# open-mmlab/Amphion

Measured on AMD Instinct MI355X. Metric: audio samples/sec (HiFi-GAN V1 22.05 kHz generator, mel->wav), higher is better.
Workload: dtype f32 (split-f16 MFMA: 3 x v_mfma_f32_32x32x16_f16 per term, f32 accumulate)

## Files before the change

amphion_amd/_lib.py:

```python
from __future__ import annotations

import ctypes
import os
import weakref
from ctypes import POINTER, c_char_p, c_float, c_int, c_int32, c_int64, c_size_t, c_void_p

_HERE = os.path.dirname(os.path.abspath(__file__))
LIB_PATH = os.environ.get("AMP_LIB_PATH") or os.path.join(_HERE, "lib", "libamphion_hip.so")

AMP_MAX_STAGES = 8
AMP_MAX_KERNELS = 8
AMP_MAX_DILATIONS = 8

AMP_ARCH_HIFIGAN, AMP_ARCH_BIGVGAN, AMP_ARCH_HIFIGAN_VITS = 0, 1, 2
AMP_ACT_LRELU, AMP_ACT_SNAKE, AMP_ACT_SNAKEBETA = 0, 1, 2
AMP_PRECISION_F32, AMP_PRECISION_F16X3 = 0, 1
AMP_CONV_OPT_PAD_REFLECT, AMP_CONV_OPT_TANH = 1, 2
AMP_PAD_REPLICATE, AMP_PAD_ZEROS, AMP_PAD_REFLECT = 0, 1, 2
AMP_PW_BIAS, AMP_PW_BIAS_GELU, AMP_PW_SCALE_RES = 0, 1, 2
PRECISIONS = {"f32": AMP_PRECISION_F32, "fp32": AMP_PRECISION_F32, "f16x3": AMP_PRECISION_F16X3}


class AmpError(RuntimeError):

# ... 109 lines not shown
    "amp_add_channel_bias": (c_int, [c_void_p, c_void_p, c_int, c_int, c_int, c_void_p]),
    "amp_layer_norm_c_ragged": (c_int, [c_void_p, c_void_p, c_void_p, c_void_p, c_void_p, c_void_p, c_int, c_int, c_int, c_float, c_int, c_void_p, c_void_p]),
    "amp_dds_seam": (c_int, [c_void_p, c_void_p, c_void_p, c_void_p, c_float, c_void_p, c_void_p, c_int, c_int, c_void_p, c_void_p, c_float,
                             c_void_p, c_int, c_int, c_int, c_void_p, c_void_p, c_void_p]),
    "amp_dwconv_layer_norm_c": (c_int, [c_void_p, c_void_p, c_void_p, c_int, c_int, c_void_p, c_void_p, c_void_p, c_int, c_int, c_int, c_float, c_int, c_void_p, c_void_p]),
    "amp_rel_attention_strided": (c_int, [c_void_p, c_void_p, c_void_p, ctypes.c_longlong, c_void_p, c_void_p, c_void_p, c_int, c_int, c_int, c_int, c_int, c_void_p, c_void_p]),
    "amp_set_rel_attention_tiled": (c_int, [c_int]),
    "amp_set_resblock_streams": (c_int, [c_int]),
    "amp_gen_prepare_streams": (c_int, [c_void_p]),
    "amp_rel_attention": (c_int, [c_void_p, c_void_p, c_void_p, c_void_p, c_void_p, c_void_p, c_int, c_int, c_int, c_int, c_int, c_void_p, c_void_p]),
    "amp_dwconv": (c_int, [c_void_p, c_void_p, c_void_p, c_void_p, c_int, c_int, c_int, c_int, c_int, c_void_p, c_void_p]),
    "amp_spline_flow": (c_int, [c_void_p, c_void_p, c_void_p, c_int, c_int, c_int, c_int, c_float, c_int, c_int, c_int, c_void_p, c_void_p]),
    "amp_spline_flow_proj": (c_int, [c_void_p, c_void_p, c_void_p, c_void_p, c_void_p, c_int, c_int, c_int, c_int, c_int, c_float, c_int, c_int, c_int, c_void_p, c_void_p]),
    "amp_affine_reverse": (c_int, [c_void_p, c_void_p, c_void_p, c_void_p, c_int, c_int, c_int, c_void_p, c_void_p]),
    "amp_embed_tokens": (c_int, [c_void_p, c_void_p, c_void_p, c_int, c_int, c_int, c_int, c_float, c_void_p, c_void_p]),
    "amp_durations": (c_int, [c_void_p, c_void_p, c_int, c_int, c_float, c_void_p, c_void_p, c_void_p, c_void_p]),
    "amp_expand_path": (c_int, [c_void_p, c_void_p, c_void_p, c_void_p, c_int, c_int, c_int, c_int, c_void_p, c_void_p, c_void_p]),
    "amp_expand_path_strided": (c_int, [c_void_p, ctypes.c_longlong, c_void_p, c_void_p, c_void_p, c_int, c_int, c_int, c_int, c_void_p, c_void_p, c_void_p]),
    "amp_gauss_sample": (c_int, [c_void_p, c_void_p, c_void_p, c_size_t, c_float, c_void_p, c_void_p]),
    "amp_snake": (c_int, [c_void_p, c_int, c_int, c_int, c_void_p, c_void_p, c_int, c_void_p, c_void_p]),
    "amp_fir_upsample": (c_int, [c_void_p, c_int, c_int, c_int, c_void_p, c_int, c_int, c_void_p, c_void_p]),
    "amp_fir_filter": (c_int, [c_void_p, c_int, c_int, c_int, c_void_p, c_int, c_int, c_int, c_int, c_int, c_void_p, c_void_p]),
    "amp_wav_to_pcm16": (c_int, [c_void_p, c_int, c_int, ctypes.c_longlong, c_void_p, c_void_p, ctypes.c_longlong, c_void_p]),
    "amp_conv_set_option": (c_int, [c_void_p, c_int, c_int]),
    "amp_pair_forward": (c_int, [c_void_p, c_void_p, c_void_p, c_int, c_int, c_float, c_void_p, c_void_p]),
    "amp_resblock_forward": (c_int, [POINTER(c_void_p), POINTER(c_void_p), c_int, c_void_p, c_int, c_int, c_float, c_void_p, c_void_p]),
    "amp_set_resblock_fusion": (c_int, [c_int]),
    "amp_conv_destroy": (None, [c_void_p]),
    "amp_set_small_conv": (c_int, [c_int]),
    "amp_set_conv_blk": (c_int, [c_int]),
    "amp_set_conv_rg_fast": (c_int, [c_int]),
    "amp_set_pingpong": (c_int, [c_int]),
    "amp_set_conv_blk_narrow": (c_int, [c_int]),
    "amp_ampblock_forward": (c_int, [POINTER(c_void_p), POINTER(c_void_p), c_int, c_void_p, c_void_p, c_int, c_void_p, c_void_p,
                                     c_void_p, c_int, c_int, c_void_p, c_int, c_float, c_void_p]),
    "amp_set_ampblock_fusion": (c_int, [c_int]),
    "amp_conv_create_gated": (c_int, [c_int, c_int, c_int, c_int, c_void_p, c_void_p, POINTER(c_void_p)]),
    "amp_wn_forward": (c_int, [POINTER(c_void_p), POINTER(c_void_p), c_int, c_void_p, c_void_p, ctypes.c_longlong, c_void_p, c_int, c_int,
                               c_void_p, c_void_p, c_void_p]),
    "amp_wn_gate": (c_int, [c_void_p, c_void_p, ctypes.c_longlong, c_void_p, c_int, c_int, c_int, c_void_p]),
    "amp_wn_accumulate": (c_int, [c_void_p, c_void_p, c_void_p, c_void_p, c_int, c_int, c_int, c_int, c_int, c_void_p]),
    "amp_sequence_mask": (c_int, [c_void_p, c_void_p, c_int, c_int, c_int, c_void_p]),
    "amp_coupling_apply": (c_int, [c_void_p, c_void_p, c_void_p, c_int, c_int, c_int, c_int, c_void_p]),
    "amp_flip_channels": (c_int, [c_void_p, c_void_p, c_int, c_int, c_int, c_void_p]),
    "amp_posterior_sample": (c_int, [c_void_p, c_void_p, c_void_p, c_void_p, c_int, c_int, c_int, c_void_p]),
    "amp_antialias_snake": (c_int, [c_void_p, c_int, c_int, c_int, c_void_p, c_void_p, c_int, c_void_p, c_void_p, c_void_p, c_void_p]),
    "amp_istft_forward": (c_int, [POINTER(amp_mel_desc), c_void_p, c_void_p, c_int, c_int, c_void_p, c_void_p, c_void_p, c_void_p, c_void_p]),
    "amp_mel_num_frames": (c_int, [POINTER(amp_mel_desc), c_int]),
    "amp_mel_init": (c_int, []),
    "amp_mel_forward_ragged": (c_int, [POINTER(amp_mel_desc), c_void_p, c_void_p, c_int, c_int, c_void_p, c_void_p, c_void_p, c_void_p, c_void_p, c_void_p, c_void_p]),
    "amp_mel_backward": (c_int, [POINTER(amp_mel_desc), c_void_p, c_int, c_int] + [c_void_p] * 11),
    "amp_mel_forward": (c_int, [POINTER(amp_mel_desc), c_void_p, c_int, c_int, c_void_p, c_void_p, c_void_p, c_void_p, c_void_p, c_void_p, c_void_p]),
}

EXPORTED_SYMBOLS = tuple(_SIGNATURES)

_lib = None


def lib():
    global _lib
    if _lib is None:
        if not os.path.exists(LIB_PATH):
            raise RuntimeError(
                f"{LIB_PATH} not found: build it with `python -m amphion_amd.build` "
                "(the HIP path has no CPU fallback)"
# ... 99 lines not shown
```

amphion_amd/build.py:

```python
from __future__ import annotations

import os
import subprocess
import sys
from concurrent.futures import ThreadPoolExecutor

HERE = os.path.dirname(os.path.abspath(__file__))
CSRC = os.path.join(HERE, "csrc")
OBJ = os.path.join(CSRC, "_build")
LIB = os.path.join(HERE, "lib", "libamphion_hip.so")
INCLUDE = os.path.join(os.path.dirname(HERE), "include")
HIPCC = os.environ.get("HIPCC", "/opt/rocm/bin/hipcc")
TAG = os.environ.get("AMP_BUILD_TAG", "")
if TAG:
    OBJ = os.path.join(CSRC, "_build_" + TAG)
    LIB = os.path.join(HERE, "lib", "libamphion_hip_" + TAG + ".so")
ARCH = "gfx950"
CONV_TAPS = (1, 2, 3, 5, 7, 11)
PAIR_TAPS = (3, 5, 7, 11)
SMALL_TAPS = (1, 3, 5, 7, 11)
BLK_TAPS = (2, 3, 7, 11)
RB_TAPS = (3, 5, 7, 11)
AMPB_TAPS = (3, 5, 7, 11)

FLAGS = ["--offload-arch=" + ARCH, "-O3", "-std=c++17", "-fPIC", "-I" + INCLUDE, "-I" + CSRC, "-Wall",
         "-Wno-unused-function"] + os.environ.get("AMP_BUILD_FLAGS", "").split()


def _units():
    units = [("runtime.hip", "runtime.o", []), ("conv_host.hip", "conv_host.o", []), ("generator.hip", "generator.o", []),
             ("ops_abi.hip", "ops_abi.o", []), ("small_kernels.hip", "small_kernels.o", []),
             ("mel.hip", "mel.o", []), ("vits_text.hip", "vits_text.o", []), ("pair3_f16x3.hip", "pair3_f16x3.o", []),
             ("conv_small3_f16x3.hip", "conv_small3_f16x3.o", []),
             ("pw_f16x3.hip", "pw_f16x3.o", []), ("dw_layer_f16x3.hip", "dw_layer_f16x3.o", []), ("diffwave.hip", "diffwave.o", [])]
    for kt in CONV_TAPS:
        units.append(("conv_mfma.hip", f"conv_mfma_kt{kt}.o", [f"-DAMP_KT={kt}"]))
        units.append(("conv_f16x3.hip", f"conv_f16x3_kt{kt}.o", [f"-DAMP_KT={kt}"]))
    for kt in BLK_TAPS:
        units.append(("conv_blk_f16x3.hip", f"conv_blk_f16x3_kt{kt}.o", [f"-DAMP_KT={kt}"]))
    for kt in SMALL_TAPS:
        units.append(("conv_small_f16x3.hip", f"conv_small_f16x3_kt{kt}.o", [f"-DAMP_KT={kt}"]))
    for kt in PAIR_TAPS:
        units.append(("pair_f16x3.hip", f"pair_f16x3_kt{kt}.o", [f"-DAMP_KT={kt}"]))
        units.append(("pair_strip_f16x3.hip", f"pair_strip_f16x3_kt{kt}.o", [f"-DAMP_KT={kt}"]))
    for kt in RB_TAPS:
        units.append(("rb_f16x3.hip", f"rb_f16x3_kt{kt}.o", [f"-DAMP_KT={kt}"]))
    for kt in AMPB_TAPS:
        units.append(("ampb_f16x3.hip", f"ampb_f16x3_kt{kt}.o", [f"-DAMP_KT={kt}"]))
    return units


def _deps_mtime():
    m = 0.0
    for root in (CSRC, INCLUDE):
        for fn in os.listdir(root):
            if fn.endswith((".h", ".hip", ".cpp")):
                m = max(m, os.path.getmtime(os.path.join(root, fn)))
    return max(m, os.path.getmtime(__file__))


def _compile(unit):
    src, obj, extra = unit
    cmd = [HIPCC] + FLAGS + extra + ["-c", os.path.join(CSRC, src), "-o", os.path.join(OBJ, obj)]
    r = subprocess.run(cmd, capture_output=True, text=True)
    if r.returncode != 0:
        raise RuntimeError("hipcc failed: " + " ".join(cmd) + "\n" + r.stdout + r.stderr)
    return obj


def build(force: bool = False, verbose: bool = False) -> str:
    os.makedirs(OBJ, exist_ok=True)
    os.makedirs(os.path.dirname(LIB), exist_ok=True)
# ... 18 lines not shown
```

amphion_amd/csrc/amp_host.h:

```cpp
#pragma once
#include <math.h>

#include <vector>

#include "amp_internal.h"

#define AMP_HIP(expr)                                                                  \
    do {                                                                               \
        hipError_t e__ = (expr);                                                       \
        if (e__ != hipSuccess) {                                                       \
            set_error("%s failed: %s (%s:%d)", #expr, hipGetErrorString(e__), __FILE__, __LINE__); \
            return AMP_ERR_HIP;                                                        \
        }                                                                              \
    } while (0)

#define AMP_RC(expr) do { int rc__ = (expr); if (rc__ != AMP_OK) return rc__; } while (0)

struct amp_conv {
    int transposed = 0, cin = 0, cout = 0, k = 0, stride = 1, dilation = 1, padding = 0;
    int M = 0, ntaps = 0, KT = 0, off0 = 0, dstep = 0, halo_left = 0, halo_right = 0, up = 1, up_pad = 0;
    int nchunks = 0;
    int precision = amp::PREC_F32;
    int pad_reflect = 0, tanh_out = 0;
    int gated_H = 0;
    int Mpad = 0;
    float wscale = 1.f;
    amp::ConvPlan plan{};
    void* wp_dev = nullptr;
    float* bias_dev = nullptr;
    ~amp_conv() {
        if (wp_dev) (void)hipFree(wp_dev);
        if (bias_dev) (void)hipFree(bias_dev);
    }
};

namespace amp {

int device_upload(const void* host, size_t bytes, void** out);

int default_precision();

constexpr int kConvBlkDefault = 3;
constexpr int kConvRgFastDefault = 1;
constexpr int kPingPongDefault = 1;
struct Config {
    int pair_strips = -1;
    int rb_fusion = 1;
    int ampb_fusion = 1;
    int conv_blk = kConvBlkDefault;
    size_t group_bytes = 0;
    int small_conv = 1;
    int conv_rg_fast = 1;
    int pingpong = 1;
    int narrow_blk = 1;
    int rb_streams = -1;
    Config();
};
Config& cfg();

struct RangeGuard {
    unsigned* dev = nullptr;
    unsigned* host = nullptr;
    hipEvent_t ev = nullptr;
    bool pending = false;
};
bool guard_init(RangeGuard& g);
void guard_free(RangeGuard& g);
int range_poll(RangeGuard* g, hipStream_t st);
int range_publish(RangeGuard* g, hipStream_t st);
int range_check_sync(RangeGuard* g, hipStream_t st, const char* who);
struct RangeFlagScope {
    explicit RangeFlagScope(unsigned* word);
    ~RangeFlagScope();
    RangeFlagScope(const RangeFlagScope&) = delete;
    RangeFlagScope& operator=(const RangeFlagScope&) = delete;
};

inline float pow2_weight_scale(float wmax) {
    int e2 = 0;
    if (wmax > 0.f) { (void)frexpf(wmax, &e2); if (ldexpf(1.f, e2 - 1) == wmax) e2 -= 1; }
    return wmax > 0.f ? ldexpf(1.f, 13 - e2) : 1.f;
}

template <class View>
std::vector<_Float16> pack_a_f16x3(int row_blocks, int k16, int taps, size_t pad_entries, float wscale, View view) {
    std::vector<_Float16> wp(((size_t)row_blocks * k16 * taps * 2 + pad_entries) * 64 * 8, (_Float16)0.f);
    for (int mb = 0; mb < row_blocks; ++mb)
// ... 46 lines not shown
```

amphion_amd/csrc/amp_internal.h:

```cpp
#pragma once
#include <hip/hip_runtime.h>
#include <stdarg.h>
#include <stdint.h>
#include <stdio.h>

#include <atomic>
#include <mutex>
#include <string>
#include <vector>

#include "amphion_hip.h"

namespace amp {

constexpr int KC = 8;
constexpr int KC16 = 16;

enum { PREC_F32 = 0, PREC_F16X3 = 1 };

struct ConvArgs {
    const float* x;
    const void* wp;
    const float* bias;
    const float* res;
    float* y;
    int B, Cin, Tin;
    long long xbs;
    int nchunks;
    int M;
    int Tq;
    int tiles_per_item;
    int rev;
    int row_groups;
    int off0, dstep;
    int halo_left;
    int wd;
    int Cout, Tout;
    int up, up_pad;
    float slope_in, slope_out;
    int mode;
    float div;
    float acc_scale, inv_scale;
    const int* lens;
    int len_mul;
    unsigned* range_flag;
    int pad_reflect;
    int tanh_out;
    int Mpad;
    const float* gate_cond;
    long long gate_cond_bs;
    int wn_H;
    float* wn_x;
    float* wn_out;
    int wn_first, wn_last;
};

struct PairArgs {
    const float* x;
    float* y;
    const void* wp1;
    const float* bias1;
    const void* wp2;
    const float* bias2;
    int B, C, T;
    int tiles_per_item;
    int strip_len;
    int strips_per_item;
    int wide;
    int rev;
    int dil;
    float slope;
    float sc1, isc1, sc2, isc2;
    int mode;
    float div;
    const int* lens;
    int len_mul;
    unsigned* range_flag;
};

struct ConvSmall3Args {
    ConvArgs a[3];
    int nx[3], ny[3];
};
hipError_t launch_conv_small3(const ConvSmall3Args& p, const int ni[3], hipStream_t stream);

struct Pair3Args {
    PairArgs a[3];
// ... 57 lines not shown
    const float* skip_in;
    float* x_out;
    float* skip_out;
    const uint4* wp1;
    const uint4* wp2;
    const float* w1f;
    const float* w2f;
    const float* bias1;
    const float* bias2;
    int C, n_mel, L, d;
    int K16;
    int tiles_per_item;
    float inv1, inv2;
    unsigned* range_flag;
};
size_t dw_layer_lds_bytes(int C, int n_mel, bool f32);
hipError_t launch_dw_layer(DwLayerArgs a, int B, bool f32, hipStream_t stream);

struct ConvPlan {
    int KT;
    int WM, WN;
    int NI;
    int HALO;
    int NT() const { return 32 * NI * WN; }
    int Mgroup() const { return 32 * WM; }
};

bool choose_plan(int ntaps, int M, int halo_total, int Tq, ConvPlan* plan);

template <int KT> hipError_t launch_conv(const ConvPlan& plan, const ConvArgs& a, hipStream_t stream);
template <int KT> hipError_t launch_conv_f16x3(const ConvPlan& plan, const ConvArgs& a, hipStream_t stream);
template <int KT> int conv_blk_nt(int cm, int halo_total);
template <int KT> hipError_t launch_conv_blk(int cm, int wn, const ConvArgs& a, hipStream_t stream);
constexpr int kSmallConvMaxChunks = 16;
template <int KT> hipError_t launch_conv_small(int ni, int epi, const ConvArgs& a, hipStream_t stream);
template <int KT> int pair_tile(int C, int dil);
template <int KT> hipError_t launch_pair(const PairArgs& a, hipStream_t stream);
template <int KT> int strip_step(int C, int dil, int wide, int* wg_per_cu);
template <int KT> hipError_t launch_strip(const PairArgs& a, hipStream_t stream);
template <int KT> int rb_tile(int C, int max_dil, int wide);
template <int KT> hipError_t launch_rb(const RbArgs& a, int wide, hipStream_t stream);
template <int KT> int ampb_tile(int C, int max_dil, int wide);
template <int KT> hipError_t launch_ampb(const AmpbArgs& a, int wide, hipStream_t stream);

hipError_t launch_conv_post(const float* x, const float* w_dev , const float* bias_dev ,
                            float* y, int B, int Cin, int T, int K, float slope_in, int apply_tanh,
                            const int* lens, int len_mul, hipStream_t stream);

hipError_t launch_act1d(const float* x, float* y, int B, int C, int T, const float* a_dev, const float* invb_dev,
                        const float* filt_up12, const float* filt_dn12, const int* lens, int len_mul,
                        hipStream_t stream, int rev = 0 );

hipError_t launch_add_channel_bias(float* y, const float* cb, int B, int C, int T, hipStream_t stream);
constexpr int AMP_MRF_MAX_PARTS = 3;
struct MrfSumArgs {
    float* y;
    const float* p[AMP_MRF_MAX_PARTS];
    int n;
    float div;
    size_t count;
};
hipError_t launch_mrf_sum(const MrfSumArgs& a, hipStream_t stream);

hipError_t launch_wn_gate(const float* a, const float* cond, long long cond_bs, float* out, int B, int H, int T,
                          hipStream_t stream);
hipError_t launch_wn_accumulate(float* x, float* out, const float* rs, const int* lens, int B, int H, int T, int last,
// ... 84 lines not shown
```

amphion_amd/csrc/conv_host.hip:

```cpp
#include <string.h>

#include <memory>
#include <type_traits>
#include <vector>

#include "amp_host.h"

namespace amp {

template <int... K> struct Taps { static constexpr int list[] = {K...}; };
using ConvTaps = Taps<1, 2, 3, 5, 7, 11>;
using BlkTaps = Taps<2, 3, 7, 11>;
using SmallTaps = Taps<1, 3, 5, 7, 11>;
using PairTaps = Taps<3, 5, 7, 11>;
using RbTaps = Taps<3, 5, 7, 11>;
using AmpbTaps = Taps<3, 5, 7, 11>;

template <int... K, typename R, typename F>
static R with_taps(Taps<K...>, int k, R dflt, F&& f) {
    R r = dflt;
    (void)((k == K && (r = f(std::integral_constant<int, K>{}), true)) || ...);
    return r;
}

static hipError_t launch_conv(const ConvPlan& p, const ConvArgs& a, hipStream_t s) {
    return with_taps(ConvTaps{}, p.KT, hipErrorInvalidValue, [&](auto K) { return launch_conv<K>(p, a, s); });
}
static hipError_t launch_conv_f16x3(const ConvPlan& p, const ConvArgs& a, hipStream_t s) {
    return with_taps(ConvTaps{}, p.KT, hipErrorInvalidValue, [&](auto K) { return launch_conv_f16x3<K>(p, a, s); });
}
static int conv_blk_nt(int k, int cm, int halo) { return with_taps(BlkTaps{}, k, 0, [&](auto K) { return conv_blk_nt<K>(cm, halo); }); }
static hipError_t launch_conv_blk(int k, int cm, int wn, const ConvArgs& a, hipStream_t s) {
    return with_taps(BlkTaps{}, k, hipErrorInvalidValue, [&](auto K) { return launch_conv_blk<K>(cm, wn, a, s); });
}
static hipError_t launch_conv_small(int k, int ni, int epi, const ConvArgs& a, hipStream_t s) {
    return with_taps(SmallTaps{}, k, hipErrorInvalidValue, [&](auto K) { return launch_conv_small<K>(ni, epi, a, s); });
}
static int pair_tile(int k, int C, int dil) { return with_taps(PairTaps{}, k, 0, [&](auto K) { return pair_tile<K>(C, dil); }); }
static hipError_t launch_pair(int k, const PairArgs& a, hipStream_t s) {
    return with_taps(PairTaps{}, k, hipErrorInvalidValue, [&](auto K) { return launch_pair<K>(a, s); });
}
static int strip_step(int k, int C, int dil, int wide, int* wg) {
    return with_taps(PairTaps{}, k, 0, [&](auto K) { return strip_step<K>(C, dil, wide, wg); });
}
static hipError_t launch_strip(int k, const PairArgs& a, hipStream_t s) {
    return with_taps(PairTaps{}, k, hipErrorInvalidValue, [&](auto K) { return launch_strip<K>(a, s); });
}
static int rb_tile(int k, int C, int max_dil, int wide) { return with_taps(RbTaps{}, k, 0, [&](auto K) { return rb_tile<K>(C, max_dil, wide); }); }
static hipError_t launch_rb(int k, const RbArgs& a, int wide, hipStream_t s) {
    return with_taps(RbTaps{}, k, hipErrorInvalidValue, [&](auto K) { return launch_rb<K>(a, wide, s); });
}
static int ampb_tile(int k, int C, int max_dil, int wide) {
    return with_taps(AmpbTaps{}, k, 0, [&](auto K) { return ampb_tile<K>(C, max_dil, wide); });
}
static hipError_t launch_ampb(int k, const AmpbArgs& a, int wide, hipStream_t s) {
    return with_taps(AmpbTaps{}, k, hipErrorInvalidValue, [&](auto K) { return launch_ampb<K>(a, wide, s); });
}

static int round_up_taps(int ntaps) {
    for (int kt : ConvTaps::list)
        if (kt >= ntaps) return kt;
    return -1;
}

bool choose_plan(int KT, int M, int halo_total, int , ConvPlan* plan) {
    bool ok = false;
// ... 24 lines not shown
        if ((long)(spi - 1) * L >= T) continue;
        const long steps = (L + hb + n1 - 1) / n1;
        const long rounds = ((long)B * spi + slots - 1) / slots;
        const long cost = rounds * (4 * steps + 1);
        if (best < 0 || cost < best) { best = cost; best_spi = spi; }
    }
    *spi_out = best_spi;
    *strip_len = (T + best_spi - 1) / best_spi;
}

static void strip_geometry(int B, int T, int n1, int hb, int wg_per_cu, int steps, bool ragged, int* strip_len, int* spi) {
    strip_plan(B, T, n1, hb, wg_per_cu, strip_len, spi);
    if (steps > 0 && steps * n1 - hb < T) { *strip_len = steps * n1 - hb; *spi = (T + *strip_len - 1) / *strip_len; }
    if (steps == 1 && !ragged && 4 * n1 - hb < T) {
        const int len4 = 4 * n1 - hb, spi4 = (T + len4 - 1) / len4;
        if ((long long)B * spi4 >= 1024) { *strip_len = len4; *spi = spi4; }
    }
}

constexpr long long kSmallGridWorkgroups = 384;

static bool small_conv_enabled() { return cfg().small_conv != 0; }

static int conv_blk_mode() { return cfg().conv_blk; }
static int narrow_blk_mode() { return cfg().narrow_blk; }
constexpr size_t kConvRgFastMaxWeightBytes = 3u << 20;
static bool conv_rg_fast() { return cfg().conv_rg_fast != 0; }
static thread_local unsigned g_launch_parity = 0;
int next_rev(const int* lens) {
    if (!cfg().pingpong || lens) return 0;
    return (int)(g_launch_parity++ & 1u);
}
constexpr long long kConvBlkMinWorkgroups = 512;

int conv_build(amp_conv* c, const float* w, const float* bias) {
    if (c->cin <= 0 || c->cout <= 0 || c->k <= 0 || c->stride <= 0 || c->dilation <= 0) {
        set_error("amp_conv: bad dimensions cin=%d cout=%d k=%d stride=%d dilation=%d", c->cin, c->cout, c->k, c->stride,
                  c->dilation);
        return AMP_ERR_INVALID;
    }
    if (!c->transposed) {
        if (c->stride != 1) { set_error("amp_conv: strided Conv1d is not on the vocoder path"); return AMP_ERR_UNSUPPORTED; }
        c->up = 1; c->up_pad = 0;
        c->M = c->cout;
        c->ntaps = c->k;
        c->off0 = -c->padding;
        c->dstep = c->dilation;
    } else if (c->stride == 1) {
        if (c->dilation != 1) { set_error("amp_conv: dilated ConvTranspose1d unsupported (dilation=%d)", c->dilation); return AMP_ERR_UNSUPPORTED; }
        c->up = 1; c->up_pad = 0;
        c->M = c->cout;
        c->ntaps = c->k;
        c->off0 = -(c->k - 1 - c->padding);
        c->dstep = 1;
    } else {
        if (c->dilation != 1) { set_error("amp_conv: dilated ConvTranspose1d unsupported (dilation=%d)", c->dilation); return AMP_ERR_UNSUPPORTED; }
        c->up = c->stride; c->up_pad = c->padding;
        c->M = c->cout * c->stride;
        c->ntaps = (c->k + c->stride - 1) / c->stride;
        c->off0 = 0;
        c->dstep = -1;
    }
    c->KT = round_up_taps(c->ntaps);
    if (c->KT < 0) { set_error("amp_conv: k=%d at stride=%d is %d taps, unsupported (max 11)", c->k, c->stride, c->ntaps); return AMP_ERR_UNSUPPORTED; }
    const int omin = c->dstep >= 0 ? c->off0 : c->off0 + (c->KT - 1) * c->dstep;
    const int omax = c->dstep >= 0 ? c->off0 + (c->KT - 1) * c->dstep : c->off0;
// ... 85 lines not shown
    a.pad_reflect = c->pad_reflect; a.tanh_out = c->tanh_out;
    a.range_flag = c->precision == PREC_F16X3 ? range_flag_for_current_device() : nullptr;
    a.rev = c->precision == PREC_F16X3 ? next_rev(lens) : 0;
    if (c->pad_reflect && (c->halo_left >= T || c->halo_right >= T)) {
        set_error("amp_conv_forward: reflection padding %d needs more than %d input samples", c->halo_left > c->halo_right ? c->halo_left : c->halo_right, T);
        return AMP_ERR_INVALID;
    }
    if (c->gated_H) { set_error("amp_conv_forward: a gated conv (amp_conv_create_gated) only runs inside amp_wn_forward"); return AMP_ERR_STATE; }
    if (c->precision == PREC_F16X3 && slope_in > 1.f) {
        set_error("amp_conv_forward: leaky_relu slope %g > 1 on the input is outside the f16x3 kernels (use AMP_PRECISION_F32)", (double)slope_in);
        return AMP_ERR_UNSUPPORTED;
    }
    tl_conv_transposed = c->transposed;
    if (c->precision == PREC_F32) {
        if (plan_small) return AMP_ERR_UNSUPPORTED;
        a.acc_scale = a.inv_scale = 1.f;
        AMP_HIP(launch_conv(plan, a, stream));
    } else {
        a.acc_scale = 16.f * c->wscale;
        a.inv_scale = 1.f / a.acc_scale;
        const long long wgs_half = (long long)B * ((a.Tq + 63) / 64) * ((c->M + plan.Mgroup() - 1) / plan.Mgroup());
        int blk_cm = 0, blk_nt = 0, blk_wn = 1;
        const bool blk_kt = c->KT == 2 || c->KT == 3 || (conv_blk_mode() == 3 && (c->KT == 7 || c->KT == 11));
        if (c->M % 256 == 0) blk_wn = 1;
        else if (c->M % 128 == 0 && c->KT != 2 && (narrow_blk_mode() >= 2 || (narrow_blk_mode() == 1 && c->KT >= 7))) blk_wn = 2;
        else blk_wn = 0;
        if (conv_blk_mode() > 0 && plan.NI == 4 && blk_wn > 0 && blk_kt && !c->tanh_out && !c->pad_reflect) {
            int cm = (conv_blk_mode() >= 2 && c->KT == 2 && c->nchunks % 2 == 0) ? 2 : 1;
            const int halo = c->halo_left + c->halo_right;
            const int nt = blk_wn * conv_blk_nt(c->KT, cm, halo);
            if (nt > 0 && (long long)B * ((a.Tq + nt - 1) / nt) * (c->M / (256 / blk_wn)) >= kConvBlkMinWorkgroups) { blk_cm = cm; blk_nt = nt; }
        }
        if (plan_small && !(blk_cm == 0 && plan.NI == 2 && small_conv_covers(c) && (c->KT <= 5 || wgs_half <= 128))) return AMP_ERR_UNSUPPORTED;
        if (blk_cm > 0) {
            const int rows = 256 / blk_wn;
            a.tiles_per_item = (a.Tq + blk_nt - 1) / blk_nt;
            a.wd = blk_nt + c->halo_left + c->halo_right;
            a.row_groups = (conv_rg_fast() && c->M / rows > 1 && conv_weight_bytes(c) <= kConvRgFastMaxWeightBytes) ? c->M / rows : 0;
            AMP_HIP(launch_conv_blk(c->KT, blk_cm, blk_wn, a, stream));
        } else if (plan.NI == 2 && small_conv_covers(c) && (c->KT <= 5 || wgs_half <= 128)) {
            const int ni = small_conv_ni(c);
            a.Mpad = c->Mpad;
            a.tiles_per_item = (a.Tq + 32 * ni - 1) / (32 * ni);
            a.wd = 32 * ni + c->halo_left + c->halo_right;
            if (plan_small) { *plan_small = a; *plan_ni = ni; return AMP_OK; }
            AMP_HIP(launch_conv_small(c->KT, ni, 0, a, stream));
        } else {
            const int nrg = (c->M + plan.Mgroup() - 1) / plan.Mgroup();
            a.row_groups = (conv_rg_fast() && nrg > 1 && conv_weight_bytes(c) <= kConvRgFastMaxWeightBytes) ? nrg : 0;
            AMP_HIP(launch_conv_f16x3(plan, a, stream));
        }
    }
    return AMP_OK;
}

bool pair_supported(const amp_conv* c1, const amp_conv* c2) {
    if (c1->precision != PREC_F16X3 || c2->precision != PREC_F16X3) return false;
    if (c1->pad_reflect || c2->pad_reflect || c1->tanh_out || c2->tanh_out) return false;
    if (c1->transposed || c2->transposed || c1->cin != c1->cout || c2->cin != c2->cout || c1->cin != c2->cin) return false;
    if (c1->k != c2->k || c2->dilation != 1 || c1->k != c1->KT) return false;
    if (c1->padding != (c1->k - 1) / 2 * c1->dilation || c2->padding != (c2->k - 1) / 2) return false;
    if (!c1->bias_dev || !c2->bias_dev) return false;
    const StripChoice sc = strip_choice(c1->cin, c1->k);
    if (sc.use && strip_step(c1->k, c1->cin, c1->dilation, sc.wide, nullptr) > 0) return true;
    return pair_tile(c1->k, c1->cin, c1->dilation) > 0;
}

// ... 450 lines not shown
```

amphion_amd/csrc/runtime.hip:

```cpp
#include <stdarg.h>
#include <stdio.h>
#include <stdlib.h>
#include <string.h>

#include <mutex>
#include <string>

#include "amp_host.h"

namespace amp {

static thread_local char g_err[512] = "";

void set_error(const char* fmt, ...) {
    va_list ap;
    va_start(ap, fmt);
    vsnprintf(g_err, sizeof(g_err), fmt, ap);
    va_end(ap);
}

static RangeGuard g_guard[64];
__thread std::string* tl_kernel_log = nullptr;
__thread char tl_last_kernel[160] = "";
__thread int tl_conv_transposed = 0;
// ... 114 lines not shown
    rb_fusion = num("AMP_RB_FUSION", 0, 3, 1);
    ampb_fusion = num("AMP_AMPB_FUSION", 0, 3, 1);
    rb_streams = num("AMP_RB_STREAMS", -1, 1, -1);
    static const char* const kRemoved[][2] = {
        {"AMP_GROUP_MB", "amp_set_group_mb(megabytes)"}, {"AMP_PAIR_STRIP", "amp_set_pair_strips(mode)"}, {"AMP_CONV_BLK", "amp_set_conv_blk(mode)"},
        {"AMP_FUSE_PAIRS", "nothing (the fused pairs are the only form)"}, {"AMP_RB_SUM_FRAMES", "nothing"},
        {"AMP_RB_HORIZONTAL", "amp_set_resblock_streams(mode)"}, {"AMP_RB_HORIZONTAL_FRAMES", "amp_set_resblock_streams(mode)"}};
    for (const auto& r : kRemoved) {
        const char* e = getenv(r[0]);
        if (e && *e) fprintf(stderr, "libamphion_hip: the environment variable %s=%s is no longer read (removed in ABI 142); use %s\n", r[0], e, r[1]);
    }
}
Config& cfg() { static Config c; return c; }

int device_upload(const void* host, size_t bytes, void** out) {
    void* p = nullptr;
    AMP_HIP(hipMalloc(&p, bytes));
    const hipError_t e = hipMemcpy(p, host, bytes, hipMemcpyHostToDevice);
    if (e != hipSuccess) {
        (void)hipFree(p);
        set_error("hipMemcpy of %zu bytes to the device failed: %s", bytes, hipGetErrorString(e));
        return AMP_ERR_HIP;
    }
    *out = p;
    return AMP_OK;
}

}

using namespace amp;

extern "C" {

int amp_version(void) { return 144; }
const char* amp_last_error(void) { return g_err; }

int amp_set_precision(int precision) {
    if (precision != AMP_PRECISION_F32 && precision != AMP_PRECISION_F16X3) {
        set_error("amp_set_precision: unknown precision %d", precision);
        return AMP_ERR_INVALID;
    }
    g_precision = precision;
    return AMP_OK;
}

int amp_get_precision(void) { return default_precision(); }

int amp_device_count(void) {
    int n = 0;
    if (hipGetDeviceCount(&n) != hipSuccess) return 0;
    return n;
}

int amp_set_pair_strips(int on) {
    if (on < -1 || on > 0) { set_error("amp_set_pair_strips: %d (-1 the policy, 0 the per-tile kernel everywhere; the four-wave strips of mode 1 left in ABI 142)", on); return AMP_ERR_INVALID; }
    cfg().pair_strips = on;
    return AMP_OK;
}

int amp_set_group_mb(int megabytes) {
    if (megabytes < 0) { set_error("amp_set_group_mb: %d", megabytes); return AMP_ERR_INVALID; }
    cfg().group_bytes = (size_t)megabytes << 20;
    return AMP_OK;
}

int amp_set_resblock_streams(int mode) {
    if (mode < -1 || mode > 1) { set_error("amp_set_resblock_streams: mode=%d", mode); return AMP_ERR_INVALID; }
    cfg().rb_streams = mode;
    return AMP_OK;
}

int amp_set_small_conv(int on) {
    cfg().small_conv = on ? 1 : 0;
    return AMP_OK;
}

int amp_set_pingpong(int on) {
    cfg().pingpong = on < 0 ? kPingPongDefault : (on ? 1 : 0);
    return AMP_OK;
}

int amp_set_conv_rg_fast(int on) {
    cfg().conv_rg_fast = on < 0 ? kConvRgFastDefault : (on ? 1 : 0);
    return AMP_OK;
}

int amp_set_conv_blk_narrow(int on) {
    if (on < -1 || on > 2) { set_error("amp_set_conv_blk_narrow: %d (0 off, 1 policy: 128-row convs with k >= 7, 2 every 128-row conv, -1 default)", on); return AMP_ERR_INVALID; }
    cfg().narrow_blk = on < 0 ? 1 : on;
    return AMP_OK;
}

int amp_set_conv_blk(int mode) {
    if (mode < -1 || mode > 3) { set_error("amp_set_conv_blk: mode %d (0 off, 1 | 2 chunks per staging round, 3 = 2 + k = 7 / 11, -1 default)", mode); return AMP_ERR_INVALID; }
    cfg().conv_blk = mode < 0 ? kConvBlkDefault : mode;
    return AMP_OK;
}

int amp_set_resblock_fusion(int mode) {
    if (mode < -1 || mode > 3) { set_error("amp_set_resblock_fusion: mode=%d", mode); return AMP_ERR_INVALID; }
    cfg().rb_fusion = mode < 0 ? 1 : mode;
    return AMP_OK;
}

int amp_set_ampblock_fusion(int mode) {
    if (mode < -1 || mode > 3) { set_error("amp_set_ampblock_fusion: mode=%d", mode); return AMP_ERR_INVALID; }
    cfg().ampb_fusion = mode < 0 ? 1 : mode;
    return AMP_OK;
}

int amp_range_check(void* stream_) {
    return range_check_sync(guard_for_current_device(), (hipStream_t)stream_, "amp_range_check");
}

}
```

include/amphion_hip.h:

```cpp
#ifndef AMPHION_HIP_H
#define AMPHION_HIP_H

#include <stddef.h>
#include <stdint.h>

#ifdef __cplusplus
extern "C" {
#endif

typedef enum amp_status {
    AMP_OK = 0,
    AMP_ERR_INVALID = -1,
    AMP_ERR_MISSING_WEIGHT = -2,
    AMP_ERR_HIP = -3,
    AMP_ERR_UNSUPPORTED = -4,
    AMP_ERR_STATE = -5,
    AMP_ERR_RANGE = -6
} amp_status;

typedef enum amp_arch {
    AMP_ARCH_HIFIGAN = 0,
    AMP_ARCH_BIGVGAN = 1,
    AMP_ARCH_HIFIGAN_VITS = 2
} amp_arch;
// ... 133 lines not shown
                            const int* ylens_dev, int B, int D, int Tx, int Ty, float* out_dev, float* attn_dev, void* stream);
int amp_gauss_sample(const float* m_dev, const float* logs_dev, const float* noise_dev, size_t n, float noise_scale,
                     float* out_dev, void* stream);

int amp_snake(const float* x_dev, int B, int C, int T, const float* alpha_dev, const float* beta_dev, int logscale,
              float* y_dev, void* stream);

int amp_wav_to_pcm16(const float* wav_dev, int B, int L, long long wav_stride, const int* lens_dev, int16_t* pcm_dev,
                     long long pcm_stride, void* stream);

typedef enum amp_conv_option { AMP_CONV_OPT_PAD_REFLECT = 1, AMP_CONV_OPT_TANH = 2 } amp_conv_option;
int amp_conv_set_option(amp_conv* c, int option, int value);

int amp_pair_forward(const amp_conv* c1, const amp_conv* c2, const float* x_dev, int B, int T, float slope,
                     float* y_dev, void* stream);

int amp_resblock_forward(const amp_conv* const* c1, const amp_conv* const* c2, int n_pairs, const float* x_dev, int B, int T,
                         float slope, float* y_dev, void* stream);
int amp_set_resblock_fusion(int mode);
int amp_set_resblock_streams(int mode);
int amp_gen_prepare_streams(amp_gen* g);

int amp_ampblock_forward(const amp_conv* const* c1, const amp_conv* const* c2, int n_pairs, const float* alpha_dev,
                         const float* beta_dev, int logscale, const float* filt_up_host, const float* filt_down_host,
                         const float* x_dev, int B, int T, float* y_dev, int mode, float div, void* stream);
int amp_set_ampblock_fusion(int mode);

void amp_conv_destroy(amp_conv* c);

int amp_set_small_conv(int on);

int amp_set_conv_blk(int mode);
int amp_set_conv_blk_narrow(int on);

int amp_set_conv_rg_fast(int on);

int amp_set_pingpong(int on);


int amp_conv_create_gated(int hidden, int k, int dilation, int padding, const float* weight_host, const float* bias_host,
                          amp_conv** out);

int amp_wn_forward(const amp_conv* const* in_layers, const amp_conv* const* res_skip_layers, int n_layers, float* x_dev,
                   const float* cond_dev, long long cond_batch_stride, const int32_t* lens_dev, int B, int T,
                   float* acts_ws_dev, float* out_dev, void* stream);


int amp_wn_gate(const float* a_dev, const float* cond_dev, long long cond_batch_stride, float* out_dev, int B, int H,
                int T, void* stream);
int amp_wn_accumulate(float* x_dev, float* out_dev, const float* rs_dev, const int32_t* lens_dev, int B, int H, int T,
                      int first, int last, void* stream);
int amp_sequence_mask(float* x_dev, const int32_t* lens_dev, int B, int C, int T, void* stream);
int amp_coupling_apply(float* x_dev, const float* m_dev, const int32_t* lens_dev, int B, int half_channels, int T,
                       int reverse, void* stream);
int amp_flip_channels(const float* x_dev, float* y_dev, int B, int C, int T, void* stream);
int amp_posterior_sample(const float* stats_dev, const float* eps_dev, const int32_t* lens_dev, float* z_dev, int B,
                         int C, int T, void* stream);

int amp_antialias_snake(const float* x_dev, int B, int C, int T, const float* alpha_dev, const float* beta_dev,
                        int logscale, const float* filt_up_host, const float* filt_down_host, float* y_dev,
                        void* stream);

typedef struct amp_mel_desc {
    uint32_t struct_size;
    int32_t n_fft;
    int32_t win_size;
// ... 76 lines not shown
```

Baseline: 151.5 million.

## Add dedicated stride-2 transposed-conv f16x3 MFMA kernel for late upsample layers

Adds a specialized kernel for stride-2, k=4 transposed convolutions with 128 or 64 input channels, the late HiFi-GAN upsample layers. It keeps the weights in registers, double-buffers the input strips in LDS with a one-column halo, and applies the LeakyReLU epilogue while writing paired output samples. A policy selects it when the tile count is large and launches a strip-tiled grid of about 1024 workgroups. The cost is another code path with a narrow shape contract and a new config knob.

```diff
diff --git a/amphion_amd/_lib.py b/amphion_amd/_lib.py
--- a/amphion_amd/_lib.py
+++ b/amphion_amd/_lib.py
@@ -165,6 +165,7 @@
     "amp_set_conv_rg_fast": (c_int, [c_int]),
     "amp_set_pingpong": (c_int, [c_int]),
     "amp_set_conv_blk_narrow": (c_int, [c_int]),
+    "amp_set_convt_form": (c_int, [c_int]),
     "amp_ampblock_forward": (c_int, [POINTER(c_void_p), POINTER(c_void_p), c_int, c_void_p, c_void_p, c_int, c_void_p, c_void_p,
                                      c_void_p, c_int, c_int, c_void_p, c_int, c_float, c_void_p]),
     "amp_set_ampblock_fusion": (c_int, [c_int]),
diff --git a/amphion_amd/build.py b/amphion_amd/build.py
--- a/amphion_amd/build.py
+++ b/amphion_amd/build.py
@@ -20,6 +20,7 @@
 PAIR_TAPS = (3, 5, 7, 11)
 SMALL_TAPS = (1, 3, 5, 7, 11)
 BLK_TAPS = (2, 3, 7, 11)
+CONVT_TAPS = (2,)
 RB_TAPS = (3, 5, 7, 11)
 AMPB_TAPS = (3, 5, 7, 11)
 
@@ -38,6 +39,8 @@
         units.append(("conv_f16x3.hip", f"conv_f16x3_kt{kt}.o", [f"-DAMP_KT={kt}"]))
     for kt in BLK_TAPS:
         units.append(("conv_blk_f16x3.hip", f"conv_blk_f16x3_kt{kt}.o", [f"-DAMP_KT={kt}"]))
+    for kt in CONVT_TAPS:
+        units.append(("convt_f16x3.hip", f"convt_f16x3_kt{kt}.o", [f"-DAMP_KT={kt}"]))
     for kt in SMALL_TAPS:
         units.append(("conv_small_f16x3.hip", f"conv_small_f16x3_kt{kt}.o", [f"-DAMP_KT={kt}"]))
     for kt in PAIR_TAPS:
diff --git a/amphion_amd/csrc/amp_host.h b/amphion_amd/csrc/amp_host.h
--- a/amphion_amd/csrc/amp_host.h
+++ b/amphion_amd/csrc/amp_host.h
@@ -43,6 +43,10 @@
 constexpr int kConvBlkDefault = 3;
 constexpr int kConvRgFastDefault = 1;
 constexpr int kPingPongDefault = 1;
+#ifndef AMP_CONVT_FORM_DEFAULT
+#define AMP_CONVT_FORM_DEFAULT 1
+#endif
+constexpr int kConvtFormDefault = AMP_CONVT_FORM_DEFAULT;
 struct Config {
     int pair_strips = -1;
     int rb_fusion = 1;
@@ -53,6 +57,7 @@
     int conv_rg_fast = 1;
     int pingpong = 1;
     int narrow_blk = 1;
+    int convt_form = kConvtFormDefault;
     int rb_streams = -1;
     Config();
 };
diff --git a/amphion_amd/csrc/amp_internal.h b/amphion_amd/csrc/amp_internal.h
--- a/amphion_amd/csrc/amp_internal.h
+++ b/amphion_amd/csrc/amp_internal.h
@@ -53,6 +53,7 @@
     float* wn_x;
     float* wn_out;
     int wn_first, wn_last;
+    int strip_tiles;
 };
 
 struct PairArgs {
@@ -176,6 +177,8 @@
 template <int KT> hipError_t launch_conv_f16x3(const ConvPlan& plan, const ConvArgs& a, hipStream_t stream);
 template <int KT> int conv_blk_nt(int cm, int halo_total);
 template <int KT> hipError_t launch_conv_blk(int cm, int wn, const ConvArgs& a, hipStream_t stream);
+template <int KT> int convt_s2_nt(int cin, int cout, int k, int stride, int padding);
+template <int KT> hipError_t launch_convt_s2(const ConvArgs& a, int strip_tiles, hipStream_t stream);
 constexpr int kSmallConvMaxChunks = 16;
 template <int KT> hipError_t launch_conv_small(int ni, int epi, const ConvArgs& a, hipStream_t stream);
 template <int KT> int pair_tile(int C, int dil);
diff --git a/amphion_amd/csrc/conv_host.hip b/amphion_amd/csrc/conv_host.hip
--- a/amphion_amd/csrc/conv_host.hip
+++ b/amphion_amd/csrc/conv_host.hip
@@ -11,6 +11,7 @@
 template <int... K> struct Taps { static constexpr int list[] = {K...}; };
 using ConvTaps = Taps<1, 2, 3, 5, 7, 11>;
 using BlkTaps = Taps<2, 3, 7, 11>;
+using ConvtTaps = Taps<2>;
 using SmallTaps = Taps<1, 3, 5, 7, 11>;
 using PairTaps = Taps<3, 5, 7, 11>;
 using RbTaps = Taps<3, 5, 7, 11>;
@@ -32,6 +33,12 @@
 static int conv_blk_nt(int k, int cm, int halo) { return with_taps(BlkTaps{}, k, 0, [&](auto K) { return conv_blk_nt<K>(cm, halo); }); }
 static hipError_t launch_conv_blk(int k, int cm, int wn, const ConvArgs& a, hipStream_t s) {
     return with_taps(BlkTaps{}, k, hipErrorInvalidValue, [&](auto K) { return launch_conv_blk<K>(cm, wn, a, s); });
+}
+static int convt_s2_nt(const amp_conv* c) {
+    return with_taps(ConvtTaps{}, c->KT, 0, [&](auto K) { return convt_s2_nt<K>(c->cin, c->cout, c->k, c->stride, c->padding); });
+}
+static hipError_t launch_convt_s2(int k, const ConvArgs& a, int strip_tiles, hipStream_t s) {
+    return with_taps(ConvtTaps{}, k, hipErrorInvalidValue, [&](auto K) { return launch_convt_s2<K>(a, strip_tiles, s); });
 }
 static hipError_t launch_conv_small(int k, int ni, int epi, const ConvArgs& a, hipStream_t s) {
     return with_taps(SmallTaps{}, k, hipErrorInvalidValue, [&](auto K) { return launch_conv_small<K>(ni, epi, a, s); });
@@ -122,6 +129,9 @@
     return (int)(g_launch_parity++ & 1u);
 }
 constexpr long long kConvBlkMinWorkgroups = 512;
+constexpr long long kConvtMinTiles = 2048;
+constexpr int kConvtWorkgroups = 1024;
+static int convt_form() { return cfg().convt_form; }
 
 int conv_build(amp_conv* c, const float* w, const float* bias) {
     if (c->cin <= 0 || c->cout <= 0 || c->k <= 0 || c->stride <= 0 || c->dilation <= 0) {
@@ -273,7 +283,13 @@
             if (nt > 0 && (long long)B * ((a.Tq + nt - 1) / nt) * (c->M / (256 / blk_wn)) >= kConvBlkMinWorkgroups) { blk_cm = cm; blk_nt = nt; }
         }
         if (plan_small && !(blk_cm == 0 && plan.NI == 2 && small_conv_covers(c) && (c->KT <= 5 || wgs_half <= 128))) return AMP_ERR_UNSUPPORTED;
-        if (blk_cm > 0) {
+        const int ct_nt = (convt_form() > 0 && !plan_small && c->transposed && !res && mode == 0 && c->KT == c->ntaps) ? convt_s2_nt(c) : 0;
+        const long long ct_tiles = ct_nt > 0 ? (long long)B * ((a.Tq + ct_nt - 1) / ct_nt) : 0;
+        if (ct_nt > 0 && (convt_form() == 2 || ct_tiles >= kConvtMinTiles)) {
+            const int tpi = (a.Tq + ct_nt - 1) / ct_nt;
+            const int spi = B >= kConvtWorkgroups ? 1 : (kConvtWorkgroups + B - 1) / B;
+            AMP_HIP(launch_convt_s2(c->KT, a, (tpi + spi - 1) / spi, stream));
+        } else if (blk_cm > 0) {
             const int rows = 256 / blk_wn;
             a.tiles_per_item = (a.Tq + blk_nt - 1) / blk_nt;
             a.wd = blk_nt + c->halo_left + c->halo_right;
diff --git a/amphion_amd/csrc/convt_f16x3.hip b/amphion_amd/csrc/convt_f16x3.hip
--- /dev/null
+++ b/amphion_amd/csrc/convt_f16x3.hip
@@ -0,0 +1,220 @@
+#include "f16x3_device.h"
+
+#ifndef AMP_KT
+#error "compile with -DAMP_KT=<taps>"
+#endif
+
+namespace amp {
+
+template <int KT, int NCH, int RB, int NI>
+__global__ __launch_bounds__(256, 2) void convt_s2_kernel(const ConvArgs a) {
+    static_assert(KT == 2, "stride 2, k = 4: two taps");
+    constexpr int WM = (NCH / 2) / RB;
+    constexpr int WN = 4 / WM;
+    constexpr int NT = 32 * NI * WN;
+    constexpr int OCT = 2 * NCH;
+    constexpr int S = NT + 1;
+    constexpr int BUF = 2 * OCT * S;
+    constexpr int NST = (OCT * NT) / 256;
+    static_assert(WM * WN == 4 && WM * RB * 2 == NCH && (OCT * NT) % 256 == 0 && (NT % 64 == 0), "tile shape");
+    extern __shared__ __attribute__((aligned(16))) uint4 smem4[];
+
+    const int tid = threadIdx.x;
+    const int lane = tid & 63;
+    const int wave = __builtin_amdgcn_readfirstlane(tid >> 6);
+    const int wm = wave / WN, wn = wave % WN;
+    const int hi = lane >> 5, l31 = lane & 31;
+
+    const int spi = (a.tiles_per_item + a.strip_tiles - 1) / a.strip_tiles;
+    const int bx = tile_order(blockIdx.x, gridDim.x, a.lens != nullptr, a.rev);
+    const int item = bx / spi;
+    const int tile0 = (bx - item * spi) * a.strip_tiles;
+    int tile1 = tile0 + a.strip_tiles < a.tiles_per_item ? tile0 + a.strip_tiles : a.tiles_per_item;
+    int Tv = a.Tin;
+    if (a.lens) {
+        const long long lv = (long long)a.lens[item] * a.len_mul;
+        const long long lim = (2 * lv + a.up_pad + 2 * NT - 1) / (2 * NT);
+        if (lim < tile1) tile1 = (int)lim;
+        Tv = lv < Tv ? (int)lv : Tv;
+    }
+    if (tile0 >= tile1) return;
+
+    Frag a_h[RB][NCH][KT], a_l[RB][NCH][KT];
+#pragma unroll
+    for (int rb = 0; rb < RB; ++rb) {
+        const uint4* wa = static_cast<const uint4*>(a.wp) + (size_t)(wm * RB + rb) * NCH * (KT * 128) + lane;
+#pragma unroll
+        for (int c = 0; c < NCH; ++c)
+#pragma unroll
+            for (int g = 0; g < KT; ++g) {
+                a_h[rb][c][g].u = wa[(c * KT + g) * 128];
+                a_l[rb][c][g].u = wa[(c * KT + g) * 128 + 64];
+            }
+    }
+    float* bsl = reinterpret_cast<float*>(smem4 + 2 * BUF);
+    if (tid < 8 * NCH) bsl[tid] = (a.bias ? a.bias[tid] : 0.f) * a.acc_scale;
+
+    const float* xb = a.x + (size_t)item * (size_t)a.xbs;
+    const float kpos = 16.f, kneg = 16.f * a.slope_in;
+    float range_max = 0.f;
+    float xs[NST][8];
+    auto stage_load = [&](int q0) {
+#pragma unroll
+        for (int it = 0; it < NST; ++it) {
+            const int ibase = wave * 64 + 256 * it;
+            const int oc = ibase / NT;
+            int t = q0 + (ibase - oc * NT) + lane;
+            t = t > a.Tin - 1 ? a.Tin - 1 : t;
+            const float* xp = xb + (size_t)(8 * oc) * a.Tin + t;
+#pragma unroll
+            for (int e = 0; e < 8; ++e) xs[it][e] = xp[(size_t)e * a.Tin];
+        }
+    };
+    auto stage_store = [&](int q0, int buf) {
+        uint4* dst = smem4 + buf * BUF;
+#pragma unroll
+        for (int it = 0; it < NST; ++it) {
+            const int ibase = wave * 64 + 256 * it;
+            const int oc = ibase / NT;
+            const int col = (ibase - oc * NT) + lane;
+            const bool tok = q0 + col < Tv;
+            uint2 h0, l0, h1, l1;
+            stage4_f16(tok ? xs[it][0] : 0.f, tok ? xs[it][1] : 0.f, tok ? xs[it][2] : 0.f, tok ? xs[it][3] : 0.f, kpos, kneg, range_max, h0, l0);
+            stage4_f16(tok ? xs[it][4] : 0.f, tok ? xs[it][5] : 0.f, tok ? xs[it][6] : 0.f, tok ? xs[it][7] : 0.f, kpos, kneg, range_max, h1, l1);
+            dst[oc * S + col + 1] = make_uint4(h0.x, h0.y, h1.x, h1.y);
+            dst[(OCT + oc) * S + col + 1] = make_uint4(l0.x, l0.y, l1.x, l1.y);
+        }
+    };
+
+    stage_load(tile0 * NT);
+    AMP_PIN_VMEM();
+    if (tid < OCT) {
+        const int t = tile0 * NT - 1;
+        const bool tok = t >= 0 && t < Tv;
+        const int tc = t < 0 ? 0 : (t > a.Tin - 1 ? a.Tin - 1 : t);
+        const float* xp = xb + (size_t)(8 * tid) * a.Tin + tc;
+        float v[8];
+#pragma unroll
+        for (int e = 0; e < 8; ++e) v[e] = tok ? xp[(size_t)e * a.Tin] : 0.f;
+        uint2 h0, l0, h1, l1;
+        stage4_f16(v[0], v[1], v[2], v[3], kpos, kneg, range_max, h0, l0);
+        stage4_f16(v[4], v[5], v[6], v[7], kpos, kneg, range_max, h1, l1);
+        smem4[tid * S] = make_uint4(h0.x, h0.y, h1.x, h1.y);
+        smem4[(OCT + tid) * S] = make_uint4(l0.x, l0.y, l1.x, l1.y);
+    }
+    stage_store(tile0 * NT, 0);
+    __syncthreads();
+
+    const float slope_out = a.slope_out;
+    const float isc = a.inv_scale;
+    struct __attribute__((packed, aligned(4))) F2 { float a, b; };
+
+    auto tile_body = [&](const int tile, const bool more) __attribute__((always_inline)) {
+        const int q0 = tile * NT;
+        const int cur = (tile - tile0) & 1;
+        if (more) {
+            stage_load(q0 + NT);
+            AMP_PIN_VMEM();
+        }
+        f32x16 acc[RB][NI];
+#pragma unroll
+        for (int rb = 0; rb < RB; ++rb)
+#pragma unroll
+            for (int t = 0; t < NI; ++t)
+#pragma unroll
+                for (int r = 0; r < 16; ++r) acc[rb][t][r] = bsl[(wm * RB + rb) * 16 + 4 * (r >> 2) + 2 * hi + ((r >> 1) & 1)];
+
+        const uint4* base = smem4 + cur * BUF + hi * S + wn * (32 * NI) + l31 + 1;
+#pragma unroll
+        for (int c = 0; c < NCH; ++c) {
+#pragma unroll
+            for (int g = 0; g < KT; ++g) {
+                const uint4* bg = base + (2 * c) * S - g;
+                Frag bh[NI], bl[NI];
+#pragma unroll
+                for (int t = 0; t < NI; ++t) {
+                    bh[t].u = bg[32 * t];
+                    bl[t].u = bg[OCT * S + 32 * t];
+                }
+#pragma unroll
+                for (int rb = 0; rb < RB; ++rb) mfma3<NI>(acc[rb], a_h[rb][c][g], a_l[rb][c][g], bh, bl);
+            }
+        }
+
+        if (more) {
+            stage_store(q0 + NT, cur ^ 1);
+            if (tid < 2 * OCT) smem4[(cur ^ 1) * BUF + tid * S] = smem4[cur * BUF + tid * S + NT];
+        }
+
+#pragma unroll
+        for (int rb = 0; rb < RB; ++rb) {
+#pragma unroll
+            for (int j = 0; j < 4; ++j) {
+#pragma unroll
+                for (int h2 = 0; h2 < 2; ++h2) {
+                    const int m0 = (wm * RB + rb) * 32 + 8 * j + 4 * hi + 2 * h2;
+                    float* yrow = a.y + ((size_t)item * a.Cout + (m0 >> 1)) * a.Tout;
+#pragma unroll
+                    for (int t = 0; t < NI; ++t) {
+                        const int q = q0 + wn * (32 * NI) + l31 + 32 * t;
+                        const int n0 = 2 * q - a.up_pad;
+                        float v0 = acc[rb][t][4 * j + 2 * h2] * isc;
+                        float v1 = acc[rb][t][4 * j + 2 * h2 + 1] * isc;
+                        v0 = v0 > 0.f ? v0 : v0 * slope_out;
+                        v1 = v1 > 0.f ? v1 : v1 * slope_out;
+                        if (q < a.Tq) {
+                            if (n0 >= 0 && n0 + 1 < a.Tout) {
+                                F2 v{v0, v1};
+                                *reinterpret_cast<F2*>(yrow + n0) = v;
+                            } else {
+                                if (n0 >= 0 && n0 < a.Tout) yrow[n0] = v0;
+                                if (n0 + 1 >= 0 && n0 + 1 < a.Tout) yrow[n0 + 1] = v1;
+                            }
+                        }
+                    }
+                }
+            }
+        }
+        __syncthreads();
+    };
+    for (int tile = tile0; tile + 1 < tile1; ++tile) tile_body(tile, true);
+    tile_body(tile1 - 1, false);
+
+    if (a.range_flag && __any(range_max > 65504.f) && lane == 0) atomicOr(a.range_flag, 1u);
+}
+
+template <int KT, int NCH, int RB, int NI>
+static hipError_t launch_one_convt(ConvArgs a, int strip_tiles, hipStream_t stream) {
+    constexpr int WN = 4 / ((NCH / 2) / RB);
+    constexpr int NT = 32 * NI * WN;
+    const size_t lds = (size_t)2 * (2 * 2 * NCH * (NT + 1)) * sizeof(uint4) + (size_t)8 * NCH * sizeof(float);
+    if (hipError_t e = ensure_dynamic_lds<&convt_s2_kernel<KT, NCH, RB, NI>>(lds); e != hipSuccess) return e;
+    a.tiles_per_item = (a.Tq + NT - 1) / NT;
+    a.strip_tiles = strip_tiles < 1 ? 1 : (strip_tiles > a.tiles_per_item ? a.tiles_per_item : strip_tiles);
+    a.wd = NT + 1;
+    a.row_groups = 0;
+    const int spi = (a.tiles_per_item + a.strip_tiles - 1) / a.strip_tiles;
+    dim3 grid((unsigned)(a.B * spi), 1u);
+    note_kernel("convt_s2_kernel", KT, NCH, RB, NI);
+    note_conv_work(a, KT, grid);
+    hipLaunchKernelGGL((convt_s2_kernel<KT, NCH, RB, NI>), grid, dim3(256), lds, stream, a);
+    return hipGetLastError();
+}
+
+template <int KT>
+int convt_s2_nt(int cin, int cout, int k, int stride, int padding) {
+    if (KT != 2 || stride != 2 || k != 4 || padding != 1 || 2 * cout != cin) return 0;
+    return cin == 128 ? 64 : cin == 64 ? 128 : 0;
+}
+
+template <int KT>
+hipError_t launch_convt_s2(const ConvArgs& a, int strip_tiles, hipStream_t stream) {
+    if (a.Cin == 128) return launch_one_convt<KT, 8, 1, 2>(a, strip_tiles, stream);
+    if (a.Cin == 64) return launch_one_convt<KT, 4, 1, 2>(a, strip_tiles, stream);
+    return hipErrorInvalidValue;
+}
+
+template int convt_s2_nt<AMP_KT>(int, int, int, int, int);
+template hipError_t launch_convt_s2<AMP_KT>(const ConvArgs&, int, hipStream_t);
+
+}
diff --git a/amphion_amd/csrc/runtime.hip b/amphion_amd/csrc/runtime.hip
--- a/amphion_amd/csrc/runtime.hip
+++ b/amphion_amd/csrc/runtime.hip
@@ -170,7 +170,7 @@
 
 extern "C" {
 
-int amp_version(void) { return 144; }
+int amp_version(void) { return 145; }
 const char* amp_last_error(void) { return g_err; }
 
 int amp_set_precision(int precision) {
@@ -235,6 +235,12 @@
     return AMP_OK;
 }
 
+int amp_set_convt_form(int mode) {
+    if (mode < -1 || mode > 2) { set_error("amp_set_convt_form: mode %d (0 off, 1 the policy, 2 every layer and grid the small-K kernel is built for, -1 default)", mode); return AMP_ERR_INVALID; }
+    cfg().convt_form = mode < 0 ? kConvtFormDefault : mode;
+    return AMP_OK;
+}
+
 int amp_set_resblock_fusion(int mode) {
     if (mode < -1 || mode > 3) { set_error("amp_set_resblock_fusion: mode=%d", mode); return AMP_ERR_INVALID; }
     cfg().rb_fusion = mode < 0 ? 1 : mode;
diff --git a/include/amphion_hip.h b/include/amphion_hip.h
--- a/include/amphion_hip.h
+++ b/include/amphion_hip.h
@@ -189,6 +189,7 @@
 
 int amp_set_conv_blk(int mode);
 int amp_set_conv_blk_narrow(int on);
+int amp_set_convt_form(int mode);
 
 int amp_set_conv_rg_fast(int on);
 
```

New measurement: 151.3 million. About the same (-0.1%).
